# abelxiaoxing/ImageClassification

Measured on AMD Instinct MI355X. Metric: images/sec (whole node) ResNet-50 bf16 224^2 training, higher is better.
Workload: dtype bf16; 1 GPU; resnet50 train step, synthetic 3x224x224, batch 256/GPU, AdamW, label smoothing 0.1, 1000 classes (BASELINE configs[1]); global_batch=256, parallelism=dp1

## Files before the change

imageclassification_amd/csrc/capi.hip:

```cpp
#include "capi_common.h"

bool g_prof_on = false;
std::vector<ProfRec> g_prof_recs;
std::vector<hipEvent_t> g_prof_pool;
hipEvent_t prof_event() {
  if (!g_prof_pool.empty()) { hipEvent_t e = g_prof_pool.back(); g_prof_pool.pop_back(); return e; }
  hipEvent_t e; (void)hipEventCreate(&e); return e;
}

extern "C" {

int icamd_abi_version(void) { return 6; }

int icamd_prof_enable(int on) { g_prof_on = on != 0; return ICAMD_OK; }
int icamd_prof_classes(void) { return PC_COUNT; }
int icamd_prof_collect(double* ms, long long* calls, double* bytes, double* flops, int n) {
  if (ms == nullptr || calls == nullptr || n < PC_COUNT) return ICAMD_ERR_BAD_ARG;
  for (auto& r : g_prof_recs) {
    (void)hipEventSynchronize(r.b);
    float t = 0.f;
    (void)hipEventElapsedTime(&t, r.a, r.b);
    ms[r.cls] += (double)t;
    calls[r.cls] += 1;
    if (bytes != nullptr) bytes[r.cls] += r.bytes;
    if (flops != nullptr) flops[r.cls] += r.flops;
    g_prof_pool.push_back(r.a);
    g_prof_pool.push_back(r.b);
  }
  g_prof_recs.clear();
  return ICAMD_OK;
}

int icamd_conv2d_stats_rows(const icamd_conv_desc* d) {
  if (!conv_desc_ok(d)) return 0;
  const long long M = (long long)d->N * d->OH * d->OW;
  return (int)((M + 127) / 128);
}

static int conv_fwd_impl(const icamd_conv_desc* d, const void* x, const void* w, void* y, const float* bias,
                         const void* addend, float* stats, int relu, void* stream, void* gelu_out = nullptr,
                         int gelu_inplace = 0) {
  if (!conv_desc_ok(d) || x == nullptr || w == nullptr || y == nullptr) return ICAMD_ERR_BAD_ARG;
  if ((long long)d->N * d->OH * d->OW >= (1ll << 31)) return ICAMD_ERR_UNSUPPORTED;
  if (d->KH == 3 && d->KW == 3 && d->stride == 1 && d->pad == 1 && addend == nullptr && gelu_out == nullptr &&
      !gelu_inplace && icamd_halo3x3_wanted(d->N, d->IH, d->IW, d->Cin, d->Cout)) {
    Halo3x3Params h;
    memset(&h, 0, sizeof(h));
    h.in = (const bf16_t*)x; h.wt = (const bf16_t*)w; h.out = (bf16_t*)y; h.bias = bias; h.stats = stats; h.relu = relu;
    h.N = d->N; h.H = d->IH; h.W = d->IW; h.C = d->Cin; h.Cout = d->Cout;
    return icamd_halo3x3_launch(h, (hipStream_t)stream);
  }
  const bool pw_gather = d->KH == 1 && d->KW == 1 && d->stride == 2 && d->pad == 0 && addend == nullptr;
  if (d->KH == 1 && d->KW == 1 && (d->stride == 1 || pw_gather) && d->pad == 0 && bias == nullptr && addend == nullptr && !relu &&
      gelu_out == nullptr && !gelu_inplace && icamd_pw_resident_wanted((long long)d->N * d->OH * d->OW, d->Cout, d->Cin)) {
    PwResidentParams g;
    memset(&g, 0, sizeof(g));
    g.A = (const bf16_t*)x; g.B = (const bf16_t*)w; g.out = (bf16_t*)y; g.stats = stats;
    g.M = d->N * d->OH * d->OW; g.N = d->Cout; g.K = d->Cin;
    if (pw_gather) { g.gat_oh = d->OH; g.gat_ow = d->OW; g.gat_ih = d->IH; g.gat_iw = d->IW; }
    return icamd_pw_resident_launch(g, (hipStream_t)stream);
  }
  if (d->KH == 1 && d->KW == 1 && (d->stride == 1 || pw_gather) && d->pad == 0 && (bias != nullptr || relu) && stats == nullptr &&
      gelu_out == nullptr && !gelu_inplace &&
      icamd_pw_resident_wanted((long long)d->N * d->OH * d->OW, d->Cout, d->Cin, addend != nullptr)) {
    PwResidentParams g;
    memset(&g, 0, sizeof(g));
    g.A = (const bf16_t*)x; g.B = (const bf16_t*)w; g.out = (bf16_t*)y; g.bias = bias; g.relu = relu;
    g.addend = (const bf16_t*)addend;
    g.M = d->N * d->OH * d->OW; g.N = d->Cout; g.K = d->Cin;
    if (pw_gather) { g.gat_oh = d->OH; g.gat_ow = d->OW; g.gat_ih = d->IH; g.gat_iw = d->IW; }
    return icamd_pw_resident_launch(g, (hipStream_t)stream);
  }
  if (d->KH == 1 && d->KW == 1 && d->stride == 1 && d->pad == 0 && addend == nullptr && !relu && stats == nullptr &&
      icamd_pw_resident_ext_wanted((long long)d->N * d->OH * d->OW, d->Cout, d->Cin)) {
    PwResidentParams g;
    memset(&g, 0, sizeof(g));
    g.A = (const bf16_t*)x; g.B = (const bf16_t*)w; g.out = (bf16_t*)y; g.bias = bias;
    g.gelu_out = (bf16_t*)gelu_out; g.gelu_inplace = gelu_inplace;
    g.M = d->N * d->OH * d->OW; g.N = d->Cout; g.K = d->Cin;
    return icamd_pw_resident_ext_launch(g, (hipStream_t)stream);
  }
  if (d->KH == 1 && d->KW == 1 && d->stride == 1 && d->pad == 0 &&
      icamd_gemm_nt_wanted((long long)d->N * d->OH * d->OW, d->Cout, d->Cin)) {
    GemmNtParams g;
    memset(&g, 0, sizeof(g));
    g.A = (const bf16_t*)x; g.B = (const bf16_t*)w; g.out = (bf16_t*)y; g.addend = (const bf16_t*)addend; g.bias = bias;
    g.stats = stats;
    g.M = d->N * d->OH * d->OW; g.N = d->Cout; g.K = d->Cin; g.relu = relu; g.gelu_out = (bf16_t*)gelu_out; g.gelu_inplace = gelu_inplace;
    return icamd_gemm_nt_launch(g, (hipStream_t)stream);
  }
  IgemmParams p;
  memset(&p, 0, sizeof(p));
  p.in = (const bf16_t*)x; p.wt = (const bf16_t*)w; p.out = (bf16_t*)y;
  p.addend = (const bf16_t*)addend; p.bias = bias; p.stats = stats; p.relu = relu; p.gelu_out = (bf16_t*)gelu_out; p.gelu_inplace = gelu_inplace;
  p.N = d->N; p.IH = d->IH; p.IW = d->IW; p.Cin = d->Cin;
  p.OH = d->OH; p.OW = d->OW; p.Cout = d->Cout;
  p.P = d->OH; p.Q = d->OW; p.M = d->N * d->OH * d->OW;
  p.ostr = 1; p.ooff_h = 0; p.ooff_w = 0; p.istr = d->stride;
  p.ntaps = d->KH * d->KW; p.Ktot = p.ntaps * d->Cin;
  p.KW = d->KW; p.pad = d->pad; p.tap_sign = 1; p.regular_taps = 1;
  if (p.ntaps <= ICAMD_MAX_TAPS)
    for (int r = 0; r < d->KH; ++r)
      for (int s = 0; s < d->KW; ++s) {
        const int t = r * d->KW + s;
        p.dh[t] = (short)(r - d->pad); p.dw[t] = (short)(s - d->pad); p.wtap[t] = (short)t;
      }
  return icamd_igemm_launch(p, (hipStream_t)stream);
}

int icamd_conv2d_fwd(const icamd_conv_desc* d, const void* x, const void* w, void* y, const float* bias,
                     const void* addend, float* stats, void* stream) {
  ProfScope _prof(PC_IGEMM_FWD, stream);
  const ConvWork cw = conv_work(d); _prof.work(cw.in + cw.out + 2 * cw.w + (addend ? cw.out : 0), cw.flops);
  return conv_fwd_impl(d, x, w, y, bias, addend, stats, 0, stream);
}

int icamd_conv2d_fwd_act(const icamd_conv_desc* d, const void* x, const void* w, void* y, const float* bias,
                         const void* addend, int relu, void* stream) {
  ProfScope _prof(PC_IGEMM_FWD, stream);
  const ConvWork cw = conv_work(d); _prof.work(cw.in + cw.out + 2 * cw.w + (addend ? cw.out : 0), cw.flops);
  return conv_fwd_impl(d, x, w, y, bias, addend, nullptr, relu ? 1 : 0, stream);
}

int icamd_conv2d_fwd_gelu(const icamd_conv_desc* d, const void* x, const void* w, void* z, void* a, const float* bias,
                          void* stream) {
  ProfScope _prof(PC_IGEMM_FWD, stream);
  const ConvWork cw = conv_work(d); _prof.work(cw.in + (z ? cw.out : 0) + cw.out + 2 * cw.w, cw.flops);
  if (a == nullptr) return ICAMD_ERR_BAD_ARG;
  if (z == nullptr) return conv_fwd_impl(d, x, w, a, bias, nullptr, nullptr, 0, stream, nullptr, 1);
  return conv_fwd_impl(d, x, w, z, bias, nullptr, nullptr, 0, stream, a);
}

static int dgrad_impl(const icamd_conv_desc* d, const void* dy, const void* w_t, void* dx, const void* addend,
                      const uint8_t* addend_bits, const icamd_bn_bwd_fuse* f, void* stream, const void* gelu_z = nullptr,
                      int addend_sub2 = 0) {
  if (!conv_desc_ok(d) || dy == nullptr || w_t == nullptr || dx == nullptr) return ICAMD_ERR_BAD_ARG;
  if (d->Cout % 8 != 0 || d->Cin % 8 != 0) return ICAMD_ERR_UNSUPPORTED;
  if ((long long)d->N * d->IH * d->IW >= (1ll << 31)) return ICAMD_ERR_UNSUPPORTED;
  const int st = d->stride;
  const bool pw_addend = icamd_pw_resident_mode() != 5;
  if (d->KH == 1 && d->KW == 1 && st == 1 && d->pad == 0 && f == nullptr && gelu_z == nullptr &&
      (addend == nullptr || pw_addend) && !(addend_bits != nullptr && addend_sub2) &&
      icamd_pw_resident_wanted((long long)d->N * d->IH * d->IW, d->Cin, d->Cout, addend != nullptr)) {
    PwResidentParams g;
    memset(&g, 0, sizeof(g));
    g.A = (const bf16_t*)dy; g.B = (const bf16_t*)w_t; g.out = (bf16_t*)dx; g.addend = (const bf16_t*)addend;
    g.addend_bits = addend_bits;
    g.M = d->N * d->IH * d->IW; g.N = d->Cin; g.K = d->Cout;
    if (addend_sub2) { g.sub2_h = d->IH; g.sub2_w = d->IW; }
    return icamd_pw_resident_launch(g, (hipStream_t)stream);
  }
  if (d->KH == 1 && d->KW == 1 && st == 1 && d->pad == 0 && f == nullptr && addend == nullptr &&
      icamd_pw_resident_ext_wanted((long long)d->N * d->IH * d->IW, d->Cin, d->Cout)) {
    PwResidentParams g;
    memset(&g, 0, sizeof(g));
    g.A = (const bf16_t*)dy; g.B = (const bf16_t*)w_t; g.out = (bf16_t*)dx; g.gelu_z = (const bf16_t*)gelu_z;
    g.M = d->N * d->IH * d->IW; g.N = d->Cin; g.K = d->Cout;
    return icamd_pw_resident_ext_launch(g, (hipStream_t)stream);
  }
  if (d->KH == 1 && d->KW == 1 && st == 1 && d->pad == 0 && f == nullptr && !(addend_bits != nullptr && addend_sub2) &&
      icamd_gemm_nt_wanted((long long)d->N * d->IH * d->IW, d->Cin, d->Cout)) {
    GemmNtParams g;
    memset(&g, 0, sizeof(g));
    g.A = (const bf16_t*)dy; g.B = (const bf16_t*)w_t; g.out = (bf16_t*)dx; g.addend = (const bf16_t*)addend;
    g.addend_bits = addend_bits;
    g.M = d->N * d->IH * d->IW; g.N = d->Cin; g.K = d->Cout; g.gelu_z = (const bf16_t*)gelu_z;
    if (addend_sub2) { g.sub2_h = d->IH; g.sub2_w = d->IW; }
    return icamd_gemm_nt_launch(g, (hipStream_t)stream);
  }
  if (d->KH == 3 && d->KW == 3 && st == 1 && d->pad == 1 && addend == nullptr && addend_bits == nullptr && f == nullptr &&
      gelu_z == nullptr && icamd_halo3x3_wanted(d->N, d->IH, d->IW, d->Cout, d->Cin)) {
    Halo3x3Params h;
    memset(&h, 0, sizeof(h));
    h.in = (const bf16_t*)dy; h.wt = (const bf16_t*)w_t; h.out = (bf16_t*)dx; h.flip = 1;
    h.N = d->N; h.H = d->IH; h.W = d->IW; h.C = d->Cout; h.Cout = d->Cin;
    return icamd_halo3x3_launch(h, (hipStream_t)stream);
  }
  float* partials = f ? f->partials : nullptr;
  for (int ph = 0; ph < st; ++ph)
    for (int pw = 0; pw < st; ++pw) {
      const int P = (d->IH - ph + st - 1) / st, Q = (d->IW - pw + st - 1) / st;
      if (P <= 0 || Q <= 0) continue;
      IgemmParams p;
      memset(&p, 0, sizeof(p));
      p.in = (const bf16_t*)dy; p.wt = (const bf16_t*)w_t; p.out = (bf16_t*)dx;
      p.addend = (const bf16_t*)addend;
      p.addend_bits = addend_bits;
      p.addend_sub2 = addend_sub2;
      p.gelu_z = (const bf16_t*)gelu_z;
      p.N = d->N; p.IH = d->OH; p.IW = d->OW; p.Cin = d->Cout;
      p.OH = d->IH; p.OW = d->IW; p.Cout = d->Cin;
      p.P = P; p.Q = Q; p.M = d->N * P * Q;
      p.ostr = st; p.ooff_h = ph; p.ooff_w = pw; p.istr = 1;
      p.Ktot = d->KH * d->KW * d->Cout;
      p.KW = d->KW; p.pad = d->pad; p.tap_sign = -1; p.regular_taps = (st == 1) ? 1 : 0;
      if (f != nullptr) {
        p.bnb_y = (const bf16_t*)f->y; p.bnb_mask = (const bf16_t*)f->mask_src;
        p.bnb_mean = f->mean; p.bnb_invstd = f->invstd; p.bnb_scale = f->scale; p.bnb_shift = f->shift;
        p.bnb_relu = f->relu; p.stats = partials;
        partials += (size_t)((p.M + 127) / 128) * 2 * d->Cin;
      }
      int nt = 0;
      for (int r = 0; r < d->KH; ++r) {
        const int eh = ph + d->pad - r;
        if (((eh % st) + st) % st != 0) continue;
        for (int s = 0; s < d->KW; ++s) {
          const int ew = pw + d->pad - s;
          if (((ew % st) + st) % st != 0) continue;
          if (nt < ICAMD_MAX_TAPS) { p.dh[nt] = (short)(eh / st); p.dw[nt] = (short)(ew / st); p.wtap[nt] = (short)(r * d->KW + s); }
          ++nt;
        }
      }
      p.ntaps = nt;
      const int rc = icamd_igemm_launch(p, (hipStream_t)stream);
      if (rc) return rc;
    }
  return ICAMD_OK;
}

int icamd_conv2d_dgrad(const icamd_conv_desc* d, const void* dy, const void* w_t, void* dx, const void* addend,
                       const uint8_t* addend_maskbits, void* stream) {
  ProfScope _prof(PC_IGEMM_DGRAD, stream);
  const ConvWork cw = conv_work(d); _prof.work(cw.out + cw.in + 2 * cw.w + (addend ? cw.in : 0) + (addend_maskbits ? cw.in / 16 : 0), cw.flops);
  if (addend_maskbits != nullptr && (addend == nullptr || d == nullptr || d->Cin % 64 != 0)) return ICAMD_ERR_BAD_ARG;
  return dgrad_impl(d, dy, w_t, dx, addend, addend_maskbits, nullptr, stream);
}

int icamd_conv2d_dgrad_sub2(const icamd_conv_desc* d, const void* dy, const void* w_t, void* dx, const void* addend_sub2,
                            void* stream) {
  ProfScope _prof(PC_IGEMM_DGRAD, stream);
  const ConvWork cw = conv_work(d); _prof.work(cw.out + cw.in + 2 * cw.w + cw.in / 4, cw.flops);
  if (addend_sub2 == nullptr) return ICAMD_ERR_BAD_ARG;
  return dgrad_impl(d, dy, w_t, dx, addend_sub2, nullptr, nullptr, stream, nullptr, 1);
}

int icamd_conv2d_dgrad_gelu(const icamd_conv_desc* d, const void* dy, const void* w_t, const void* z, void* dz,
                            void* stream) {
  ProfScope _prof(PC_IGEMM_DGRAD, stream);
  const ConvWork cw = conv_work(d); _prof.work(cw.out + 2 * cw.in + 2 * cw.w, cw.flops);
  if (z == nullptr) return ICAMD_ERR_BAD_ARG;
  return dgrad_impl(d, dy, w_t, dz, nullptr, nullptr, nullptr, stream, z);
}

int icamd_conv2d_dgrad_stats_rows(const icamd_conv_desc* d) {
  if (!conv_desc_ok(d)) return 0;
  int rows = 0;
  for (int ph = 0; ph < d->stride; ++ph)
    for (int pw = 0; pw < d->stride; ++pw) {
      const long long P = (d->IH - ph + d->stride - 1) / d->stride, Q = (d->IW - pw + d->stride - 1) / d->stride;
      if (P > 0 && Q > 0) rows += (int)((d->N * P * Q + 127) / 128);
    }
  return rows;
}

int icamd_conv2d_dgrad_bnbwd(const icamd_conv_desc* d, const void* dy, const void* w_t, void* g, const void* addend,
                             const icamd_bn_bwd_fuse* f, void* stream) {
  ProfScope _prof(PC_IGEMM_DGRAD, stream);
  const ConvWork cw = conv_work(d); _prof.work(cw.out + 2 * cw.in + 2 * cw.w + (addend ? cw.in : 0), cw.flops);
  if (f == nullptr || f->y == nullptr || f->mean == nullptr || f->invstd == nullptr || f->partials == nullptr)
    return ICAMD_ERR_BAD_ARG;
  return dgrad_impl(d, dy, w_t, g, addend, nullptr, f, stream);
}

int icamd_conv2d_dgrad_bnred_supported(const icamd_conv_desc* d) {
  if (!conv_desc_ok(d) || d->KH != 1 || d->KW != 1 || d->stride != 1 || d->pad != 0) return 0;
  return icamd_pw_resident_bnred_wanted((long long)d->N * d->IH * d->IW, d->Cin, d->Cout) ? 1 : 0;
}

int icamd_conv2d_dgrad_bnred(const icamd_conv_desc* d, const void* dy, const void* w_t, void* g, const void* addend,
                             const uint8_t* addend_bits, int addend_sub2, const void* bn_y, const uint8_t* bn_bits,
                             float* partials, void* stream) {
  ProfScope _prof(PC_IGEMM_DGRAD, stream);
  const ConvWork cw = conv_work(d); _prof.work(cw.out + 3 * cw.in + 2 * cw.w + cw.in / 16 + (addend_bits ? cw.in / 16 : 0), cw.flops);
  if (!conv_desc_ok(d) || dy == nullptr || w_t == nullptr || g == nullptr || addend == nullptr || bn_y == nullptr ||
      bn_bits == nullptr || partials == nullptr || (addend_sub2 && addend_bits != nullptr))
    return ICAMD_ERR_BAD_ARG;
  if (!icamd_conv2d_dgrad_bnred_supported(d)) return ICAMD_ERR_UNSUPPORTED;
  PwResidentParams p;
  memset(&p, 0, sizeof(p));
  p.A = (const bf16_t*)dy; p.B = (const bf16_t*)w_t; p.out = (bf16_t*)g; p.addend = (const bf16_t*)addend;
  p.addend_bits = addend_bits;
  p.bn_y = (const bf16_t*)bn_y; p.bn_bits = bn_bits; p.bn_part = partials;
  p.M = d->N * d->IH * d->IW; p.N = d->Cin; p.K = d->Cout;
  if (addend_sub2) { p.sub2_h = d->IH; p.sub2_w = d->IW; }
  return icamd_pw_resident_bnred_launch(p, (hipStream_t)stream);
}

size_t icamd_conv2d_wgrad_workspace_bytes(const icamd_conv_desc* d) {
  if (!conv_desc_ok(d)) return 0;
  int S = 1, rows = 0;
  const long long M = (long long)d->N * d->OH * d->OW;
  if (M >= (1ll << 30)) return 0;
  const int Ktot = d->KH * d->KW * d->Cin;
  icamd_wgrad_plan((int)M, d->Cout, Ktot, &S, &rows);
  if (icamd_wgrad_halo_wanted(d->KH, d->KW, d->stride, d->pad, d->OH, d->OW, d->Cin, d->Cout, M)) {
    int S2 = 1;
    icamd_wgrad_halo_plan((int)M, d->Cin, d->Cout, &S2, &rows);
    if (S2 > S) S = S2;
  }
  return wgrad_ws(nullptr, S, d->Cout, Ktot).bytes;
}

static int wgrad_impl(const icamd_conv_desc* d, const void* x, const void* dy, float* dw, float* dbias, int accumulate,
                      void* workspace, size_t workspace_bytes, void* stream);

int icamd_conv2d_wgrad(const icamd_conv_desc* d, const void* x, const void* dy, float* dw, int accumulate,
                       void* workspace, size_t workspace_bytes, void* stream) {
  ProfScope _prof(PC_WGRAD, stream);
  const ConvWork cw = conv_work(d); _prof.work(cw.in + cw.out + 4 * cw.w, cw.flops);
  return wgrad_impl(d, x, dy, dw, nullptr, accumulate, workspace, workspace_bytes, stream);
}

int icamd_conv2d_wgrad_bias(const icamd_conv_desc* d, const void* x, const void* dy, float* dw, float* dbias,
                            int accumulate, void* workspace, size_t workspace_bytes, void* stream) {
  ProfScope _prof(PC_WGRAD, stream);
  const ConvWork cw = conv_work(d); _prof.work(cw.in + cw.out + 4 * cw.w, cw.flops);
  if (dbias == nullptr) return ICAMD_ERR_BAD_ARG;
  return wgrad_impl(d, x, dy, dw, dbias, accumulate, workspace, workspace_bytes, stream);
}

static int wgrad_impl(const icamd_conv_desc* d, const void* x, const void* dy, float* dw, float* dbias, int accumulate,
                      void* workspace, size_t workspace_bytes, void* stream) {
  if (!conv_desc_ok(d) || x == nullptr || dy == nullptr || dw == nullptr || workspace == nullptr) return ICAMD_ERR_BAD_ARG;
  const size_t need = icamd_conv2d_wgrad_workspace_bytes(d);
  if (need == 0 || workspace_bytes < need) return ICAMD_ERR_WORKSPACE;
  WgradParams p;
  memset(&p, 0, sizeof(p));
  p.x = (const bf16_t*)x; p.dy = (const bf16_t*)dy; p.slab = (float*)workspace;
  p.N = d->N; p.IH = d->IH; p.IW = d->IW; p.Cin = d->Cin; p.OH = d->OH; p.OW = d->OW; p.Cout = d->Cout;
// ... 19 lines not shown
```

imageclassification_amd/csrc/conv3x3_halo.hip:

```cpp
#ifndef ICAMD_C64_NT
#define ICAMD_C64_NT 0
#endif
#include "common.h"
#include "icamd_internal.h"
#include <cstdlib>

namespace {

template <int N> __device__ __forceinline__ void halo_wait_vmcnt() {
  static_assert(N >= 0 && N < 64, "vmcnt is a 6-bit field");
  asm volatile("s_waitcnt vmcnt(%0)" ::"n"(N) : "memory");
}

__device__ __forceinline__ int swzq(int blk) { return (0x78 >> (2 * blk)) & 3; }

template <int BN, int WN, int MFR, int LA, int NB, int KS, int WPS>
__global__ __launch_bounds__(256, WPS) void conv3x3_halo_kernel(const Halo3x3Params p) {
  constexpr int WM = 4 / WN;
  constexpr int BM = WM * MFR * 16;
  constexpr int NJ = BN / WN / 16;
  constexpr int A_SLOTS = 4 * LA * 8;
  constexpr int ZERO_SLOT = A_SLOTS - 1;
  constexpr int A_BYTES = A_SLOTS * 128;
  constexpr int B_STAGE = BN * KS * 2;
  constexpr int LB = BN * KS / 2048;
  static_assert(KS == 32 || KS == 64, "filter stage width");
  constexpr int RING = NB * B_STAGE;
  constexpr int EPI_BYTES = BM * BN * 2;
  constexpr int LDS_BYTES = (A_BYTES + RING > EPI_BYTES) ? A_BYTES + RING : EPI_BYTES;
  static_assert(NB >= 2 && NB <= 8 && (WN == 1 || WN == 2) && LB >= 1, "configuration");
  __shared__ __attribute__((aligned(16))) unsigned char smem[LDS_BYTES];
  unsigned char* const sA = smem;
  unsigned char* const sB = smem + A_BYTES;

  const int tid = threadIdx.x, lane = tid & 63;
  const int wave = __builtin_amdgcn_readfirstlane(tid >> 6);
  const int wm = wave % WM, wn = wave / WM;
  const int fr = lane & 15, fq = lane >> 4;

  const unsigned int nblk = gridDim.x;
  unsigned int L;
  {
    const unsigned int xcd = blockIdx.x & 7u, idx = blockIdx.x >> 3;
    const unsigned int q = nblk >> 3, r = nblk & 7u;
    L = (xcd < r ? xcd * (q + 1) : r * (q + 1) + (xcd - r) * q) + idx;
  }
  const int tile_m = L / p.ntiles_n, tile_n = L - tile_m * p.ntiles_n;
  const int m0 = tile_m * BM, n0 = tile_n * BN;
  const int W = p.W, C = p.C;
  const bf16_t* __restrict__ in = p.in;
  const bf16_t* __restrict__ wt = p.wt;
  const bf16_t* zero = (const bf16_t*)icamd_zero_page;

  const int a_slot_lane = lane >> 3;
  int b_src[LB];
#pragma unroll
  for (int j = 0; j < LB; ++j) {
    int row, lc;
    if constexpr (KS == 64) {
      row = (wave * LB + j) * 8 + (lane >> 3);
      lc = ((lane & 7) ^ ((row >> 1) & 7)) * 8;
    } else {
      row = (wave * LB + j) * 16 + (lane >> 2);
      lc = ((lane & 3) ^ swzq((row >> 2) & 3)) * 8;
    }
    const int co = n0 + row;
    b_src[j] = (co < p.Cout) ? co * 9 * C + lc : -1;
  }
  auto stage_a = [&](int slice) {
#pragma unroll
    for (int j = 0; j < LA; ++j) {
      const int slot = (wave * LA + j) * 8 + a_slot_lane;
      const int pix = m0 - (W + 1) + slot;
      const int lc = (((lane & 7) - slot) & 7) * 8;
      const bf16_t* src = (pix >= 0 && pix < p.M && slot != ZERO_SLOT) ? in + ((long long)pix * C + slice * 64 + lc) : zero;
      __builtin_amdgcn_global_load_lds(GPTR(src), LPTR(sA + (wave * LA + j) * 1024), 16, 0, 0);
    }
  };
  auto stage_b = [&](int slice, int tap, int kk, int slot) {
    const int wtap = p.flip ? 8 - tap : tap;
    const int off = wtap * C + slice * 64 + kk * 32;
#pragma unroll
    for (int j = 0; j < LB; ++j) {
      const bf16_t* src = b_src[j] >= 0 ? wt + (b_src[j] + off) : zero;
      __builtin_amdgcn_global_load_lds(GPTR(src), LPTR(sB + slot * B_STAGE + (wave * LB + j) * 1024), 16, 0, 0);
    }
  };

  int slot0[MFR];
  unsigned int vmask[MFR];
#pragma unroll
  for (int i = 0; i < MFR; ++i) {
    const int ml = wm * (BM / WM) + i * 16 + fr;
    const int m = m0 + ml;
    slot0[i] = ml + W + 1;
    unsigned int mk = 0;
    if (m < p.M) {
      const unsigned int n = fdiv((unsigned)m, p.divHW);
      const unsigned int rem = m - n * (p.H * W);
      const int h = (int)fdiv(rem, p.divW);
      const int w = (int)(rem - (unsigned)h * W);
#pragma unroll
      for (int t = 0; t < 9; ++t) {
        const int dh = t / 3 - 1, dw = t % 3 - 1;
        if ((unsigned)(h + dh) < (unsigned)p.H && (unsigned)(w + dw) < (unsigned)W) mk |= 1u << t;
      }
    }
    vmask[i] = mk;
  }
  f32x4 acc[NJ][MFR];
#pragma unroll
  for (int j = 0; j < NJ; ++j)
#pragma unroll
    for (int i = 0; i < MFR; ++i) acc[j][i] = f32x4{0.f, 0.f, 0.f, 0.f};

  const int nslices = C >> 6;
  constexpr int SPT = 64 / KS;
  const int nstages = nslices * 9 * SPT;
  stage_a(0);
  int issue_q = 0, issue_slice = 0, issue_tap = 0, issue_kk = 0, fill = 0;
  auto issue_b = [&]() {
    stage_b(issue_slice, issue_tap, issue_kk, fill);
    fill = fill == NB - 1 ? 0 : fill + 1;
    ++issue_q;
    if (++issue_kk == SPT) {
      issue_kk = 0;
      if (++issue_tap == 9) { issue_tap = 0; ++issue_slice; }
    }
  };
#pragma unroll
  for (int k = 0; k < NB - 1; ++k)
    if (issue_q < nstages) issue_b();

  const int b_row = wn * (BN / WN) + fr;
  const int b_frag = KS == 64 ? b_row * 128 : b_row * 64 + ((fq ^ swzq((fr >> 2) & 3)) << 4);
  const int bsw = (fr >> 1) & 7;
  int read = 0, q = 0;
  for (int slice = 0; slice < nslices; ++slice) {
#pragma unroll 1
    for (int tap = 0; tap < 9; ++tap) {
      const int trow = tap >= 6 ? 2 : (tap >= 3 ? 1 : 0);
      const int doff = (trow - 1) * W + (tap - 3 * trow - 1);
      const unsigned int tbit = 1u << tap;
      int aaddr[MFR];
#pragma unroll
      for (int i = 0; i < MFR; ++i) {
        const int sl = (vmask[i] & tbit) ? slot0[i] + doff : ZERO_SLOT;
        aaddr[i] = sl * 128 + (((fq + sl) & 7) << 4);
      }
#pragma unroll
      for (int st = 0; st < SPT; ++st, ++q) {
        {
          const int younger = issue_q - 1 - q;
          if (younger >= 4) halo_wait_vmcnt<4 * LB>();
          else if (younger == 3) halo_wait_vmcnt<3 * LB>();
          else if (younger == 2) halo_wait_vmcnt<2 * LB>();
          else if (younger == 1) halo_wait_vmcnt<LB>();
          else halo_wait_vmcnt<0>();
        }
        asm volatile("s_waitcnt lgkmcnt(0)" ::: "memory");
        __builtin_amdgcn_s_barrier();
        if (issue_q < nstages) issue_b();
        const unsigned char* sb = sB + read * B_STAGE + b_frag;
        read = read == NB - 1 ? 0 : read + 1;
#pragma unroll
        for (int kk = (KS == 64 ? 0 : st); kk < (KS == 64 ? 2 : st + 1); ++kk) {
          bf16x8 wf[NJ];
#pragma unroll
          for (int j = 0; j < NJ; ++j) {
            if constexpr (KS == 64) wf[j] = *(const bf16x8*)(sb + j * 2048 + (((kk * 4 + fq) ^ bsw) << 4));
            else wf[j] = *(const bf16x8*)(sb + j * 1024);
          }
#pragma unroll
          for (int i = 0; i < MFR; ++i) {
            const bf16x8 xf = *(const bf16x8*)(sA + (kk ? (aaddr[i] ^ 64) : aaddr[i]));
#pragma unroll
            for (int j = 0; j < NJ; ++j) acc[j][i] = __builtin_amdgcn_mfma_f32_16x16x32_bf16(wf[j], xf, acc[j][i], 0, 0, 0);
          }
        }
      }
    }
    if (slice + 1 < nslices) {
      asm volatile("s_waitcnt lgkmcnt(0)" ::: "memory");
      __builtin_amdgcn_s_barrier();
      stage_a(slice + 1);
      halo_wait_vmcnt<0>();
    }
  }
  __syncthreads();

  constexpr int ROWB = BN * 2, CPR = BN / 8;
#pragma unroll
  for (int j = 0; j < NJ; ++j) {
    const int cl = wn * (BN / WN) + j * 16 + 4 * fq;
    const int cg = n0 + cl;
    const int cgc = cg < p.Cout ? cg : 0;
    f32x4 b4 = {0.f, 0.f, 0.f, 0.f};
    if (p.bias != nullptr) b4 = *(const f32x4*)(p.bias + cgc);
#pragma unroll
    for (int i = 0; i < MFR; ++i) {
      const int ml = wm * (BM / WM) + i * 16 + fr;
      f32x4 v = acc[j][i] + b4;
      if (p.relu) {
#pragma unroll
        for (int e = 0; e < 4; ++e) v[e] = v[e] < 0.f ? 0.f : v[e];
      }
      u32x2 pk;
      pk[0] = pack_bf16x2(v[0], v[1]);
      pk[1] = pack_bf16x2(v[2], v[3]);
      const int slot = cl >> 2;
      *(u32x2*)(smem + ml * ROWB + ((((slot >> 1) ^ ml) & (CPR - 1)) << 4) + ((slot & 1) << 3)) = pk;
    }
  }
  __syncthreads();
  constexpr int RPP = 256 / CPR;
  constexpr int NPASS = BM / RPP;
  const int cp = tid & (CPR - 1), rg = tid / CPR;
  const int co = n0 + cp * 8;
  const bool co_ok = co < p.Cout;
  float s1[8], s2[8];
#pragma unroll
  for (int e = 0; e < 8; ++e) { s1[e] = 0.f; s2[e] = 0.f; }
#pragma unroll
  for (int ps = 0; ps < NPASS; ++ps) {
    const int ml = ps * RPP + rg;
    const int m = m0 + ml;
    const u32x4 o = *(const u32x4*)(smem + ml * ROWB + (((cp ^ ml) & (CPR - 1)) << 4));
    if (m < p.M && co_ok) {
      *(u32x4*)(p.out + (long long)m * p.Cout + co) = o;
      if (p.stats != nullptr) {
#pragma unroll
        for (int e = 0; e < 4; ++e) {
          const float lo = bf16_lo(o[e]), hi = bf16_hi(o[e]);
          s1[2 * e] += lo; s2[2 * e] += lo * lo;
          s1[2 * e + 1] += hi; s2[2 * e + 1] += hi * hi;
        }
      }
    }
  }
  if (p.stats != nullptr) {
    __syncthreads();
    float* red = (float*)smem;
#pragma unroll
    for (int e = 0; e < 8; ++e) {
      red[(rg * 2 + 0) * BN + cp * 8 + e] = s1[e];
      red[(rg * 2 + 1) * BN + cp * 8 + e] = s2[e];
    }
    __syncthreads();
    const int ntm = (p.M + BM - 1) / BM, nrows = (p.M + 127) / 128;
    for (int idx = tid; idx < 2 * BN; idx += 256) {
      const int which = idx / BN, c = idx - which * BN;
      float s = 0.f;
#pragma unroll 4
      for (int g = 0; g < RPP; ++g) s += red[(g * 2 + which) * BN + c];
      if (n0 + c < p.Cout) {
        p.stats[((long long)tile_m * 2 + which) * p.Cout + n0 + c] = s;
        if (ntm + tile_m < nrows) p.stats[((long long)(ntm + tile_m) * 2 + which) * p.Cout + n0 + c] = 0.f;
      }
    }
  }
}

template <bool ACT>
__global__ __launch_bounds__(256, 2) void conv3x3_c64_resident_kernel(const Halo3x3Params p, const int ntiles) {
  constexpr int BM = 128, LA = 8;
  constexpr int A_BYTES = 32 * LA * 128;
  constexpr int E_BYTES = 4 * 64 * 64;
  constexpr int ZERO_SLOT = 32 * LA - 1;
  __shared__ __attribute__((aligned(16))) unsigned char smem[2 * A_BYTES + E_BYTES];

  const int tid = threadIdx.x, lane = tid & 63;
  const int wave = __builtin_amdgcn_readfirstlane(tid >> 6);
  const int wm = wave & 1, wn = wave >> 1;
  const int fr = lane & 15, fq = lane >> 4;
  const int W = p.W, H = p.H;
  const bf16_t* __restrict__ in = p.in;
  const bf16_t* zero = (const bf16_t*)icamd_zero_page;
  unsigned char* const sE = smem + 2 * A_BYTES + wave * 4096;
  const unsigned lds_base = (unsigned)(uintptr_t)LPTR(smem);

  const int a_slot = wave * 8 + (lane >> 3);
  const int a_lc = (((lane & 7) - (lane >> 3)) & 7) * 8;
  const bool a_zero_lane = a_slot == 31;
  auto stage_a = [&](int m0, unsigned char* dst) {
    const int pix0 = m0 - (W + 1) + a_slot;
    const bf16_t* src0 = in + ((long long)pix0 * 64 + a_lc);
    if (m0 - (W + 1) >= 0 && m0 - (W + 1) + LA * 32 <= p.M) {
#pragma unroll
      for (int j = 0; j < LA; ++j) {
        const bf16_t* src = src0 + j * (32 * 64);
        if (j == LA - 1) src = a_zero_lane ? zero : src;
        __builtin_amdgcn_global_load_lds(GPTR(src), LPTR(dst + (j * 4 + wave) * 1024), 16, 0, ICAMD_C64_NT);
      }
    } else {
#pragma unroll
      for (int j = 0; j < LA; ++j) {
        const int pix = pix0 + j * 32;
        const bf16_t* src = (pix >= 0 && pix < p.M && !(j == LA - 1 && a_zero_lane)) ? src0 + j * (32 * 64) : zero;
        __builtin_amdgcn_global_load_lds(GPTR(src), LPTR(dst + (j * 4 + wave) * 1024), 16, 0, ICAMD_C64_NT);
      }
    }
  };

  int buf = 0;
  int tile = blockIdx.x;
  if (tile < ntiles) stage_a(tile * BM, smem);

  bf16x8 wf[18][2];
#pragma unroll
  for (int ks = 0; ks < 18; ++ks) {
    const int tap = ks >> 1;
    const int wtap = p.flip ? 8 - tap : tap;
#pragma unroll
    for (int j = 0; j < 2; ++j)
      wf[ks][j] = *(const bf16x8*)(p.wt + ((wn * 32 + j * 16 + fr) * 9 + wtap) * 64 + (ks & 1) * 32 + fq * 8);
  }
  __builtin_amdgcn_s_waitcnt(0x0F70);

  f32x2 s1[4], s2[4];
#pragma unroll
  for (int e = 0; e < 4; ++e) { s1[e] = f32x2{0.f, 0.f}; s2[e] = f32x2{0.f, 0.f}; }

  for (; tile < ntiles; tile += gridDim.x, buf ^= 1) {
    const int m0 = tile * BM;
    halo_wait_vmcnt<4>();
    asm volatile("s_waitcnt lgkmcnt(0)" ::: "memory");
    __builtin_amdgcn_s_barrier();
    if (tile + (int)gridDim.x < ntiles) stage_a((tile + gridDim.x) * BM, smem + (buf ^ 1) * A_BYTES);

    const unsigned sa = lds_base + (unsigned)(buf * A_BYTES);
    const unsigned zaddr = sa + (unsigned)(ZERO_SLOT * 128);
    unsigned abase[3];
    bool hv0[4], hv2[4], wv0[4], wv2[4];
    {
      const int ml0 = wm * 64 + fr;
#pragma unroll
      for (int d = 0; d < 3; ++d) {
        const int sl = ml0 + d;
        abase[d] = sa + (unsigned)((sl << 7) | (((fq + sl) & 7) << 4));
      }
#pragma unroll
      for (int i = 0; i < 4; ++i) {
        unsigned int m = (unsigned)(m0 + ml0 + i * 16);
        if (m >= (unsigned)p.M) m = 0;
        const unsigned int n = fdiv(m, p.divHW);
        const unsigned int rem = m - n * (H * W);
        const int h = (int)fdiv(rem, p.divW);
        const int w = (int)(rem - (unsigned)h * W);
        hv0[i] = h > 0; hv2[i] = h + 1 < H; wv0[i] = w > 0; wv2[i] = w + 1 < W;
      }
    }
    f32x4 acc[2][4];
#pragma unroll
    for (int j = 0; j < 2; ++j)
#pragma unroll
      for (int i = 0; i < 4; ++i) acc[j][i] = f32x4{0.f, 0.f, 0.f, 0.f};

    bf16x8 xf[2][4];
    unsigned aaddr[4];
    auto tap_addresses = [&](int tap) {
      const int dh = tap / 3, dw = tap % 3;
      const unsigned t = abase[dw] + (unsigned)(dh * W * 128);
#pragma unroll
      for (int i = 0; i < 4; ++i) {
        const bool okh = dh == 0 ? hv0[i] : (dh == 2 ? hv2[i] : true);
        const bool okw = dw == 0 ? wv0[i] : (dw == 2 ? wv2[i] : true);
        aaddr[i] = (okh && okw) ? t : zaddr - (unsigned)(i * 2048);
      }
    };
#define ICAMD_READ4(dst, X)                                                                      \
  asm volatile("ds_read_b128 %0, %1" : "=v"(dst[0]) : "v"(aaddr[0] ^ (X)));                      \
  asm volatile("ds_read_b128 %0, %1 offset:2048" : "=v"(dst[1]) : "v"(aaddr[1] ^ (X)));          \
  asm volatile("ds_read_b128 %0, %1 offset:4096" : "=v"(dst[2]) : "v"(aaddr[2] ^ (X)));          \
  asm volatile("ds_read_b128 %0, %1 offset:6144" : "=v"(dst[3]) : "v"(aaddr[3] ^ (X)));
    tap_addresses(0);
    ICAMD_READ4(xf[0], 0u)
#pragma unroll
    for (int ks = 0; ks < 18; ++ks) {
      asm volatile("s_waitcnt lgkmcnt(0)"
                   : "+v"(xf[ks & 1][0]), "+v"(xf[ks & 1][1]), "+v"(xf[ks & 1][2]), "+v"(xf[ks & 1][3])::"memory");
      if (ks + 1 < 18) {
        if (((ks + 1) & 1) == 0) {
          tap_addresses((ks + 1) >> 1);
          ICAMD_READ4(xf[(ks + 1) & 1], 0u)
        } else {
          ICAMD_READ4(xf[(ks + 1) & 1], 64u)
        }
      }
      __builtin_amdgcn_sched_barrier(0);
#pragma unroll
      for (int i = 0; i < 4; ++i)
#pragma unroll
        for (int j = 0; j < 2; ++j)
          acc[j][i] = __builtin_amdgcn_mfma_f32_16x16x32_bf16(wf[ks][j], xf[ks & 1][i], acc[j][i], 0, 0, 0);
    }
#undef ICAMD_READ4

#pragma unroll
    for (int j = 0; j < 2; ++j) {
      f32x4 b4 = {0.f, 0.f, 0.f, 0.f};
      if constexpr (ACT) {
        if (p.bias != nullptr) b4 = *(const f32x4*)(p.bias + wn * 32 + j * 16 + 4 * fq);
      }
#pragma unroll
      for (int i = 0; i < 4; ++i) {
        const int pl = i * 16 + fr;
        f32x4 v = acc[j][i];
        if constexpr (ACT) {
          v += b4;
          if (p.relu) {
#pragma unroll
            for (int e = 0; e < 4; ++e) v[e] = v[e] < 0.f ? 0.f : v[e];
          }
        }
        u32x2 pk;
        pk[0] = pack_bf16x2(v[0], v[1]);
        pk[1] = pack_bf16x2(v[2], v[3]);
        const int slot = j * 4 + fq;
        *(u32x2*)(sE + pl * 64 + ((((slot >> 1) ^ (pl >> 2)) & 3) << 4) + ((slot & 1) << 3)) = pk;
      }
    }
    {
      const int pl0 = lane >> 2;
      const int mrow = m0 + wm * 64 + pl0;
      bf16_t* orow = p.out + ((long long)mrow * 64 + wn * 32 + (lane & 3) * 8);
      const bool want_stats = p.stats != nullptr;
#pragma unroll
      for (int r = 0; r < 4; ++r) {
        const int pl = r * 16 + pl0;
        const u32x4 o = *(const u32x4*)(sE + pl * 64 + ((((lane & 3) ^ (pl >> 2)) & 3) << 4));
        if (mrow + r * 16 < p.M) {
          *(u32x4*)(orow + r * (16 * 64)) = o;
          if (want_stats) {
#pragma unroll
            for (int e = 0; e < 4; ++e) {
              const f32x2 v = {bf16_lo(o[e]), bf16_hi(o[e])};
              s1[e] += v;
              s2[e] = __builtin_elementwise_fma(v, v, s2[e]);
            }
          }
        }
      }
    }
  }

  if (p.stats != nullptr) {
    __syncthreads();
    float* red = (float*)smem;
    const int g = wm * 16 + (lane >> 2);
    const int c0 = wn * 32 + (lane & 3) * 8;
#pragma unroll
    for (int e = 0; e < 4; ++e) {
      red[(g * 2 + 0) * 64 + c0 + 2 * e] = s1[e][0];
      red[(g * 2 + 0) * 64 + c0 + 2 * e + 1] = s1[e][1];
      red[(g * 2 + 1) * 64 + c0 + 2 * e] = s2[e][0];
      red[(g * 2 + 1) * 64 + c0 + 2 * e + 1] = s2[e][1];
    }
    __syncthreads();
    if (tid < 128) {
      const int which = tid >> 6, c = tid & 63;
      float s = 0.f;
#pragma unroll 8
      for (int k = 0; k < 32; ++k) s += red[(k * 2 + which) * 64 + c];
      p.stats[((long long)blockIdx.x * 2 + which) * 64 + c] = s;
      const int nrows = (p.M + 127) / 128;
      for (int r = blockIdx.x + gridDim.x; r < nrows; r += gridDim.x) p.stats[((long long)r * 2 + which) * 64 + c] = 0.f;
    }
  }
}

int launch_resident_c64(const Halo3x3Params& p, hipStream_t stream) {
  const int ntiles = (p.M + 127) / 128;
  const int slots = 2 * icamd_num_cus();
  const int grid = ntiles < slots ? ntiles : slots;
  if (p.bias != nullptr || p.relu)
    hipLaunchKernelGGL((conv3x3_c64_resident_kernel<true>), dim3((unsigned)grid), dim3(256), 0, stream, p, ntiles);
  else
    hipLaunchKernelGGL((conv3x3_c64_resident_kernel<false>), dim3((unsigned)grid), dim3(256), 0, stream, p, ntiles);
  return icamd_launch_status();
}

template <int BN, int WN, int MFR, int LA, int NB, int KS, int WPS>
int launch_halo(const Halo3x3Params& p, hipStream_t stream) {
  constexpr int BM = (4 / WN) * MFR * 16;
  const int ntm = (p.M + BM - 1) / BM;
  hipLaunchKernelGGL((conv3x3_halo_kernel<BN, WN, MFR, LA, NB, KS, WPS>), dim3((unsigned)(ntm * p.ntiles_n)), dim3(256), 0,
                     stream, p);
  return icamd_launch_status();
}

int halo_mode() {
  static const int m = icamd_env_int("ICAMD_CONV3X3_HALO", 1);
  return m;
}

}

static bool resident_c64_ok(int W, int C, int Cout) {
  static const int on = icamd_env_int("ICAMD_CONV3X3_RESIDENT", 1);
  return on != 0 && C == 64 && Cout == 64 && W % 8 == 0 && 128 + 2 * W + 2 <= 255;
}

bool icamd_halo3x3_wanted(int N, int H, int W, int C, int Cout) {
  if (halo_mode() == 0) return false;
  if (C % 64 != 0 || Cout % 8 != 0 || W < 3 || H < 3) return false;
  if (resident_c64_ok(W, C, Cout)) return true;
  if (halo_mode() == 1 && C < 256) return false;
  if ((long long)N * H * W >= (1ll << 30)) return false;
  if (2 * W + 3 + 128 > 4 * 8 * 8) return false;
  return true;
}

int icamd_halo3x3_launch(Halo3x3Params& p, hipStream_t stream) {
  if (!icamd_halo3x3_wanted(p.N, p.H, p.W, p.C, p.Cout)) return ICAMD_ERR_UNSUPPORTED;
  p.M = p.N * p.H * p.W;
  p.divHW = make_fastdiv((unsigned)(p.H * p.W));
  p.divW = make_fastdiv((unsigned)p.W);
  if (resident_c64_ok(p.W, p.C, p.Cout)) return launch_resident_c64(p, stream);
  const int bn = p.Cout <= 64 ? 64 : 128;
  p.ntiles_n = (p.Cout + bn - 1) / bn;
  int bm = 128;
  if (halo_mode() == 3) bm = 256;
  else if (halo_mode() != 2) {
    long long best = -1;
    for (int cand : {256, 224, 128}) {
      if (cand == 224 && bn != 128) continue;
      if ((cand + 2 * p.W + 3 + 31) / 32 > (cand == 128 ? 8 : 12)) continue;
      const long long tiles = (long long)((p.M + cand - 1) / cand) * p.ntiles_n;
      const long long cost = ((tiles + 511) / 512) * cand + (cand == 128 ? 16 : 0);
      if (best < 0 || cost < best) { best = cost; bm = cand; }
    }
  }
  const bool big = bm != 128;
  const int slots = bm + 2 * p.W + 2 + 1;
  const int la = (slots + 31) / 32;
  if (la > 12) return ICAMD_ERR_UNSUPPORTED;
  if (bn == 128) {
    if (bm == 224) {
      if (la <= 8) return launch_halo<128, 2, 7, 8, 3, 64, 2>(p, stream);
      if (la <= 10) return launch_halo<128, 2, 7, 10, 2, 64, 2>(p, stream);
      return launch_halo<128, 2, 7, 12, 2, 64, 2>(p, stream);
    }
    if (big) {
      if (la <= 9) return launch_halo<128, 2, 8, 9, 2, 64, 2>(p, stream);
      if (la <= 10) return launch_halo<128, 2, 8, 10, 2, 64, 2>(p, stream);
      return launch_halo<128, 2, 8, 12, 2, 64, 2>(p, stream);
    }
    if (la <= 5) return launch_halo<128, 2, 4, 5, 3, 64, 2>(p, stream);
    if (la <= 6) return launch_halo<128, 2, 4, 6, 3, 64, 2>(p, stream);
    return launch_halo<128, 2, 4, 8, 3, 64, 2>(p, stream);
  }
  if (big) {
    if (la <= 9) return launch_halo<64, 1, 4, 9, 6, 32, 2>(p, stream);
    if (la <= 10) return launch_halo<64, 1, 4, 10, 6, 32, 2>(p, stream);
    return launch_halo<64, 1, 4, 12, 6, 32, 2>(p, stream);
  }
  if (la <= 5) return launch_halo<64, 1, 2, 5, 6, 32, 3>(p, stream);
  if (la <= 6) return launch_halo<64, 1, 2, 6, 6, 32, 3>(p, stream);
  return launch_halo<64, 1, 2, 8, 6, 32, 2>(p, stream);
}
```

imageclassification_amd/csrc/icamd_internal.h:

```cpp
#pragma once
#include "common.h"

#define ICAMD_MAX_TAPS 56

struct IgemmParams {
  const bf16_t* in;
  const bf16_t* wt;
  bf16_t* out;
  const bf16_t* addend;
  const unsigned char* addend_bits;
  int addend_sub2;
  const float* bias;
  float* stats;
  const bf16_t* bnb_y;
  const bf16_t* bnb_mask;
  const float *bnb_mean, *bnb_invstd, *bnb_scale, *bnb_shift;
  int bnb_relu;
  int relu;
  bf16_t* gelu_out;
  int gelu_inplace;
  const bf16_t* gelu_z;
  int N, IH, IW, Cin;
  int OH, OW, Cout;
  int P, Q, M;
  int ostr, ooff_h, ooff_w, istr;
  int ntaps, Ktot;
  int KW, pad;
  int tap_sign, regular_taps;
  int stem7;
  int ksteps, ntiles_n;
  FastDiv divPQ, divQ, divCin, divKW;
  short dh[ICAMD_MAX_TAPS], dw[ICAMD_MAX_TAPS], wtap[ICAMD_MAX_TAPS];
};
int icamd_igemm_launch(IgemmParams& p, hipStream_t stream);
int icamd_igemm_pick_bn(int Cout);

struct Halo3x3Params {
  const bf16_t* in;
  const bf16_t* wt;
  bf16_t* out;
  const float* bias;
  float* stats;
  int relu;
  int flip;
  int N, H, W, C, Cout;
  int M, ntiles_n;
  FastDiv divHW, divW;
};
bool icamd_halo3x3_wanted(int N, int H, int W, int C, int Cout);
int icamd_halo3x3_launch(Halo3x3Params& p, hipStream_t stream);

struct GConvParams {
  const bf16_t* in;
  const bf16_t* w;
  bf16_t* out;
  const bf16_t* dy;
  float* slab;
  const float* bias;
  float* stats;
  int relu;
  int N, IH, IW, OH, OW, C, groups, stride;
  int Cg, M, npix_in, nalloc;
  int S, tiles_per_split, ntiles;
  FastDiv divOHW, divOW;
};
bool icamd_gconv3x3_ok(int N, int IH, int IW, int OH, int OW, int C, int groups, int stride);
int icamd_gconv3x3_fwd_launch(GConvParams& p, hipStream_t stream);
int icamd_gconv3x3_dgrad_launch(GConvParams& p, hipStream_t stream);
size_t icamd_gconv3x3_wgrad_bytes(int N, int IH, int IW, int OH, int OW, int C, int groups, int stride);
int icamd_gconv3x3_wgrad_launch(GConvParams& p, hipStream_t stream);

struct Pool2x2Params {
  const bf16_t* in;
  const bf16_t* addend;
  bf16_t* out;
  int N, IH, IW, C8;
  int OH, OW;
  unsigned int total;
  FastDiv divC8, divOW, divOH;
};
bool icamd_avgpool2x2_ok(int N, int IH, int IW, int C);
int icamd_avgpool2x2_launch(Pool2x2Params& p, int backward, hipStream_t stream);

struct ThinConvParams {
  const bf16_t* in;
  const bf16_t* w;
  bf16_t* out;
  const bf16_t* dy;
  float* slab;
  const float* bias;
  float* stats;
  int relu;
  int N, H, W, Cout;
  int M, nalloc, ntiles;
  int S, tiles_per_split;
  FastDiv divHW, divW;
};
bool icamd_thin3x3_ok(int N, int H, int W, int Cin, int Cout);
int icamd_thin3x3_stats_rows(int N, int H, int W, int Cout);
int icamd_thin3x3_fwd_launch(ThinConvParams& p, hipStream_t stream);
int icamd_thin3x3_dgrad_launch(ThinConvParams& p, hipStream_t stream);
size_t icamd_thin3x3_wgrad_bytes(int N, int H, int W, int Cout);
int icamd_thin3x3_wgrad_launch(ThinConvParams& p, hipStream_t stream);

struct GemmNtParams {
  const bf16_t* A;
  const bf16_t* B;
  bf16_t* out;
  const bf16_t* addend;
  const unsigned char* addend_bits;
  const float* bias;
  float* stats;
  int M, N, K;
  int sub2_h, sub2_w;
  FastDiv divHW, divW;
  int relu;
  bf16_t* gelu_out;
  int gelu_inplace;
  const bf16_t* gelu_z;
  int ntiles_n;
  int group_n;
  int out_policy;
};
int icamd_gemm_nt_launch(GemmNtParams& p, hipStream_t stream);
bool icamd_gemm_nt_wanted(long long M, int N, int K);

struct PwResidentParams {
  const bf16_t* A;
  const bf16_t* B;
  bf16_t* out;
  const bf16_t* addend;
  const unsigned char* addend_bits;
  float* stats;
  int M, N, K;
  int sub2_h, sub2_w;
  FastDiv divHW, divW;
  int rows_per_split, ntiles_n;
  int xcd_groups;
  int nt_loads;
  const bf16_t* bn_y;
  const unsigned char* bn_bits;
  float* bn_part;
  int lda, Ktrue;
  const float* bias;
  int relu;
  bf16_t* gelu_out;
  int gelu_inplace;
  const bf16_t* gelu_z;
  int gat_oh, gat_ow, gat_ih, gat_iw;
  FastDiv gdivHW, gdivW;
};
bool icamd_pw_resident_wanted(long long M, int N, int K, bool with_addend = false);
int icamd_pw_resident_mode();
bool icamd_pw_resident_ext_wanted(long long M, int N, int K);
int icamd_pw_resident_launch(PwResidentParams& p, hipStream_t stream);
int icamd_pw_resident_ext_launch(PwResidentParams& p, hipStream_t stream);
bool icamd_pw_resident_bnred_wanted(long long M, int N, int K);
int icamd_pw_resident_bnred_launch(PwResidentParams& p, hipStream_t stream);

struct StemParams {
  const bf16_t* x;
  const bf16_t* w;
  bf16_t* y;
  float* stats;
  int N, H, W, OH, OW;
  const float* bias;
  int relu;
};
struct StemWgradParams {
  const bf16_t* x;
  const bf16_t* dy;
  float* slab;
  int N, H, W, OH, OW;
};
bool icamd_stem_resident_wanted(int N, int H, int W, int Cout);
int icamd_stem_wgrad_resident_splits(int N, int H);
int icamd_stem_wgrad_resident_launch(StemWgradParams& p, int S, hipStream_t stream);
int icamd_stem_resident_launch(StemParams& p, hipStream_t stream);

struct FusedBwdParams {
  const bf16_t* g;
  const bf16_t* y;
  const bf16_t* x;
  const bf16_t* wt;
  bf16_t* dx;
  float* slab;
  const float *mean, *invstd, *scale, *c1, *c2;
  int M, CI, CO;
  int S, rows_per_split, nslices, xcd_pairs, nt;
};
bool icamd_conv1x1_bn_bwd_fused_wanted(long long M, int Cin, int Cout);
void icamd_conv1x1_bn_bwd_fused_plan(int M, int Cin, int* S, int* rows_per_split);
int icamd_conv1x1_bn_bwd_fused_launch(FusedBwdParams& p, hipStream_t stream);

struct FusedFwdParams {
  const bf16_t* y;
  const bf16_t* res;
  const float *scale, *shift, *res_scale, *res_shift;
  bf16_t* out;
  unsigned char* maskbits;
  const bf16_t* w;
  bf16_t* y1;
  float* stats;
// ... 186 lines not shown
```

Measured before the change: 14710 images/sec.

## Add sub-pixel halo kernel for stride-2 3x3 conv data gradient

Routes stride-2 3x3 conv dgrad through the halo-tiled conv kernel using a sub-pixel (phase) decomposition. Each of the four output parity classes uses only the 1, 2 or 4 filter taps that contribute to it, and results are scattered to interleaved output rows. This replaces four separate strided implicit-GEMM launches with one launch that skips zero taps and reuses the halo staging path. The new template branch adds index math in the epilogue, and correctness depends on the tap/parity mapping.

Result: no change. 14780 images/sec (median of 6 runs) (+0.5%).

```diff
diff --git a/imageclassification_amd/csrc/capi.hip b/imageclassification_amd/csrc/capi.hip
--- a/imageclassification_amd/csrc/capi.hip
+++ b/imageclassification_amd/csrc/capi.hip
@@ -175,6 +175,15 @@
     h.in = (const bf16_t*)dy; h.wt = (const bf16_t*)w_t; h.out = (bf16_t*)dx; h.flip = 1;
     h.N = d->N; h.H = d->IH; h.W = d->IW; h.C = d->Cout; h.Cout = d->Cin;
     return icamd_halo3x3_launch(h, (hipStream_t)stream);
+  }
+  if (d->KH == 3 && d->KW == 3 && st == 2 && d->pad == 1 && d->IH % 2 == 0 && d->IW % 2 == 0 && addend == nullptr &&
+      addend_bits == nullptr && f == nullptr && gelu_z == nullptr &&
+      icamd_halo3x3_s2dgrad_wanted(d->N, d->OH, d->OW, d->Cout, d->Cin)) {
+    Halo3x3Params h;
+    memset(&h, 0, sizeof(h));
+    h.in = (const bf16_t*)dy; h.wt = (const bf16_t*)w_t; h.out = (bf16_t*)dx;
+    h.N = d->N; h.H = d->OH; h.W = d->OW; h.C = d->Cout; h.Cout = d->Cin;
+    return icamd_halo3x3_s2dgrad_launch(h, (hipStream_t)stream);
   }
   float* partials = f ? f->partials : nullptr;
   for (int ph = 0; ph < st; ++ph)
diff --git a/imageclassification_amd/csrc/conv3x3_halo.hip b/imageclassification_amd/csrc/conv3x3_halo.hip
--- a/imageclassification_amd/csrc/conv3x3_halo.hip
+++ b/imageclassification_amd/csrc/conv3x3_halo.hip
@@ -14,7 +14,7 @@
 
 __device__ __forceinline__ int swzq(int blk) { return (0x78 >> (2 * blk)) & 3; }
 
-template <int BN, int WN, int MFR, int LA, int NB, int KS, int WPS>
+template <int BN, int WN, int MFR, int LA, int NB, int KS, int WPS, int S2D = 0>
 __global__ __launch_bounds__(256, WPS) void conv3x3_halo_kernel(const Halo3x3Params p) {
   constexpr int WM = 4 / WN;
   constexpr int BM = WM * MFR * 16;
@@ -38,10 +38,17 @@
   const int wm = wave % WM, wn = wave / WM;
   const int fr = lane & 15, fq = lane >> 4;
 
-  const unsigned int nblk = gridDim.x;
+  unsigned int nblk = gridDim.x, bid = blockIdx.x;
+  int pa = 0, pb = 0;
+  if constexpr (S2D) {
+    nblk >>= 2;
+    const unsigned int cls = bid / nblk;
+    bid -= cls * nblk;
+    pa = (int)(3u - cls) >> 1; pb = (int)(3u - cls) & 1;
+  }
   unsigned int L;
   {
-    const unsigned int xcd = blockIdx.x & 7u, idx = blockIdx.x >> 3;
+    const unsigned int xcd = bid & 7u, idx = bid >> 3;
     const unsigned int q = nblk >> 3, r = nblk & 7u;
     L = (xcd < r ? xcd * (q + 1) : r * (q + 1) + (xcd - r) * q) + idx;
   }
@@ -71,14 +78,19 @@
 #pragma unroll
     for (int j = 0; j < LA; ++j) {
       const int slot = (wave * LA + j) * 8 + a_slot_lane;
-      const int pix = m0 - (W + 1) + slot;
+      const int pix = S2D ? m0 + slot : m0 - (W + 1) + slot;
       const int lc = (((lane & 7) - slot) & 7) * 8;
-      const bf16_t* src = (pix >= 0 && pix < p.M && slot != ZERO_SLOT) ? in + ((long long)pix * C + slice * 64 + lc) : zero;
+      const bool live = S2D ? slot < BM + W + 2 : slot != ZERO_SLOT;
+      const bf16_t* src = (pix >= 0 && pix < p.M && live) ? in + ((long long)pix * C + slice * 64 + lc) : zero;
       __builtin_amdgcn_global_load_lds(GPTR(src), LPTR(sA + (wave * LA + j) * 1024), 16, 0, 0);
     }
   };
   auto stage_b = [&](int slice, int tap, int kk, int slot) {
-    const int wtap = p.flip ? 8 - tap : tap;
+    int wtap = p.flip ? 8 - tap : tap;
+    if constexpr (S2D) {
+      const int dq = pb ? (tap & 1) : 0, dp = pb ? (tap >> 1) : tap;
+      wtap = (pa ? (dp ? 0 : 2) : 1) * 3 + (pb ? (dq ? 0 : 2) : 1);
+    }
     const int off = wtap * C + slice * 64 + kk * 32;
 #pragma unroll
     for (int j = 0; j < LB; ++j) {
@@ -93,17 +105,21 @@
   for (int i = 0; i < MFR; ++i) {
     const int ml = wm * (BM / WM) + i * 16 + fr;
     const int m = m0 + ml;
-    slot0[i] = ml + W + 1;
+    slot0[i] = S2D ? ml : ml + W + 1;
     unsigned int mk = 0;
     if (m < p.M) {
       const unsigned int n = fdiv((unsigned)m, p.divHW);
       const unsigned int rem = m - n * (p.H * W);
       const int h = (int)fdiv(rem, p.divW);
       const int w = (int)(rem - (unsigned)h * W);
-#pragma unroll
-      for (int t = 0; t < 9; ++t) {
-        const int dh = t / 3 - 1, dw = t % 3 - 1;
-        if ((unsigned)(h + dh) < (unsigned)p.H && (unsigned)(w + dw) < (unsigned)W) mk |= 1u << t;
+      if constexpr (S2D) {
+        mk = 1u | (w + 1 < W ? 2u : 0u) | (h + 1 < p.H ? 4u : 0u);
+      } else {
+#pragma unroll
+        for (int t = 0; t < 9; ++t) {
+          const int dh = t / 3 - 1, dw = t % 3 - 1;
+          if ((unsigned)(h + dh) < (unsigned)p.H && (unsigned)(w + dw) < (unsigned)W) mk |= 1u << t;
+        }
       }
     }
     vmask[i] = mk;
@@ -116,7 +132,8 @@
 
   const int nslices = C >> 6;
   constexpr int SPT = 64 / KS;
-  const int nstages = nslices * 9 * SPT;
+  const int ntaps = S2D ? (1 + pa) * (1 + pb) : 9;
+  const int nstages = nslices * ntaps * SPT;
   stage_a(0);
   int issue_q = 0, issue_slice = 0, issue_tap = 0, issue_kk = 0, fill = 0;
   auto issue_b = [&]() {
@@ -125,7 +142,7 @@
     ++issue_q;
     if (++issue_kk == SPT) {
       issue_kk = 0;
-      if (++issue_tap == 9) { issue_tap = 0; ++issue_slice; }
+      if (++issue_tap == ntaps) { issue_tap = 0; ++issue_slice; }
     }
   };
 #pragma unroll
@@ -138,14 +155,23 @@
   int read = 0, q = 0;
   for (int slice = 0; slice < nslices; ++slice) {
 #pragma unroll 1
-    for (int tap = 0; tap < 9; ++tap) {
-      const int trow = tap >= 6 ? 2 : (tap >= 3 ? 1 : 0);
-      const int doff = (trow - 1) * W + (tap - 3 * trow - 1);
-      const unsigned int tbit = 1u << tap;
+    for (int tap = 0; tap < ntaps; ++tap) {
+      int doff;
+      unsigned int tbit;
+      if constexpr (S2D) {
+        const int dq = pb ? (tap & 1) : 0, dp = pb ? (tap >> 1) : tap;
+        doff = dp * W + dq;
+        tbit = 1u | (dq ? 2u : 0u) | (dp ? 4u : 0u);
+      } else {
+        const int trow = tap >= 6 ? 2 : (tap >= 3 ? 1 : 0);
+        doff = (trow - 1) * W + (tap - 3 * trow - 1);
+        tbit = 1u << tap;
+      }
       int aaddr[MFR];
 #pragma unroll
       for (int i = 0; i < MFR; ++i) {
-        const int sl = (vmask[i] & tbit) ? slot0[i] + doff : ZERO_SLOT;
+        const bool ok = S2D ? (vmask[i] & tbit) == tbit : (vmask[i] & tbit) != 0;
+        const int sl = ok ? slot0[i] + doff : ZERO_SLOT;
         aaddr[i] = sl * 128 + (((fq + sl) & 7) << 4);
       }
 #pragma unroll
@@ -227,7 +253,15 @@
     const int m = m0 + ml;
     const u32x4 o = *(const u32x4*)(smem + ml * ROWB + (((cp ^ ml) & (CPR - 1)) << 4));
     if (m < p.M && co_ok) {
-      *(u32x4*)(p.out + (long long)m * p.Cout + co) = o;
+      long long orow = m;
+      if constexpr (S2D) {
+        const unsigned int n = fdiv((unsigned)m, p.divHW);
+        const unsigned int rem = m - n * (p.H * W);
+        const int h = (int)fdiv(rem, p.divW);
+        const int w = (int)(rem - (unsigned)h * W);
+        orow = ((long long)n * (2 * p.H) + (2 * h + pa)) * (2 * W) + (2 * w + pb);
+      }
+      *(u32x4*)(p.out + orow * p.Cout + co) = o;
       if (p.stats != nullptr) {
 #pragma unroll
         for (int e = 0; e < 4; ++e) {
@@ -480,12 +514,12 @@
   return icamd_launch_status();
 }
 
-template <int BN, int WN, int MFR, int LA, int NB, int KS, int WPS>
+template <int BN, int WN, int MFR, int LA, int NB, int KS, int WPS, int S2D = 0>
 int launch_halo(const Halo3x3Params& p, hipStream_t stream) {
   constexpr int BM = (4 / WN) * MFR * 16;
   const int ntm = (p.M + BM - 1) / BM;
-  hipLaunchKernelGGL((conv3x3_halo_kernel<BN, WN, MFR, LA, NB, KS, WPS>), dim3((unsigned)(ntm * p.ntiles_n)), dim3(256), 0,
-                     stream, p);
+  hipLaunchKernelGGL((conv3x3_halo_kernel<BN, WN, MFR, LA, NB, KS, WPS, S2D>),
+                     dim3((unsigned)(ntm * p.ntiles_n) * (S2D ? 4u : 1u)), dim3(256), 0, stream, p);
   return icamd_launch_status();
 }
 
@@ -559,3 +593,55 @@
   if (la <= 6) return launch_halo<64, 1, 2, 6, 6, 32, 3>(p, stream);
   return launch_halo<64, 1, 2, 8, 6, 32, 2>(p, stream);
 }
+
+bool icamd_halo3x3_s2dgrad_wanted(int N, int P, int Q, int C, int Cout) {
+  if (halo_mode() == 0) return false;
+  if (C % 64 != 0 || Cout % 8 != 0 || P < 1 || Q < 1) return false;
+  if ((long long)N * P * Q >= (1ll << 28)) return false;
+  if (128 + Q + 3 > 4 * 8 * 8) return false;
+  return true;
+}
+
+int icamd_halo3x3_s2dgrad_launch(Halo3x3Params& p, hipStream_t stream) {
+  if (!icamd_halo3x3_s2dgrad_wanted(p.N, p.H, p.W, p.C, p.Cout) || p.stats != nullptr || p.bias != nullptr || p.relu)
+    return ICAMD_ERR_UNSUPPORTED;
+  p.M = p.N * p.H * p.W;
+  p.divHW = make_fastdiv((unsigned)(p.H * p.W));
+  p.divW = make_fastdiv((unsigned)p.W);
+  const int bn = p.Cout <= 64 ? 64 : 128;
+  p.ntiles_n = (p.Cout + bn - 1) / bn;
+  int bm = 128;
+  if (halo_mode() == 3) bm = 256;
+  else if (halo_mode() != 2) {
+    long long best = -1;
+    for (int cand : {256, 224, 128}) {
+      if (cand == 224 && bn != 128) continue;
+      if ((cand + p.W + 3 + 31) / 32 > (cand == 128 ? 8 : 12)) continue;
+      const long long tiles = (long long)((p.M + cand - 1) / cand) * p.ntiles_n;
+      long long rounds = (9 * tiles + 511) / 512;
+      if (rounds < 4) rounds = 4;
+      const long long cost = rounds * cand + (cand == 128 ? 16 : 0);
+      if (best < 0 || cost < best) { best = cost; bm = cand; }
+    }
+  }
+  const int la = (bm + p.W + 2 + 1 + 31) / 32;
+  if (la > (bm == 128 ? 8 : 12)) return ICAMD_ERR_UNSUPPORTED;
+  if (bn == 128) {
+    if (bm == 224) {
+      if (la <= 8) return launch_halo<128, 2, 7, 8, 3, 64, 2, 1>(p, stream);
+      return launch_halo<128, 2, 7, 12, 2, 64, 2, 1>(p, stream);
+    }
+    if (bm == 256) {
+      if (la <= 9) return launch_halo<128, 2, 8, 9, 2, 64, 2, 1>(p, stream);
+      return launch_halo<128, 2, 8, 12, 2, 64, 2, 1>(p, stream);
+    }
+    if (la <= 5) return launch_halo<128, 2, 4, 5, 3, 64, 2, 1>(p, stream);
+    return launch_halo<128, 2, 4, 8, 3, 64, 2, 1>(p, stream);
+  }
+  if (bm == 256) {
+    if (la <= 9) return launch_halo<64, 1, 4, 9, 6, 32, 2, 1>(p, stream);
+    return launch_halo<64, 1, 4, 12, 6, 32, 2, 1>(p, stream);
+  }
+  if (la <= 5) return launch_halo<64, 1, 2, 5, 6, 32, 3, 1>(p, stream);
+  return launch_halo<64, 1, 2, 8, 6, 32, 2, 1>(p, stream);
+}
diff --git a/imageclassification_amd/csrc/icamd_internal.h b/imageclassification_amd/csrc/icamd_internal.h
--- a/imageclassification_amd/csrc/icamd_internal.h
+++ b/imageclassification_amd/csrc/icamd_internal.h
@@ -49,6 +49,8 @@
 };
 bool icamd_halo3x3_wanted(int N, int H, int W, int C, int Cout);
 int icamd_halo3x3_launch(Halo3x3Params& p, hipStream_t stream);
+bool icamd_halo3x3_s2dgrad_wanted(int N, int P, int Q, int C, int Cout);
+int icamd_halo3x3_s2dgrad_launch(Halo3x3Params& p, hipStream_t stream);
 
 struct GConvParams {
   const bf16_t* in;
```
